# AnimatedRNG/alphazero-rs

Hardware: AMD Instinct MI355X
Metric: selfplay_games_per_sec (higher is better)
Workload: dtype bf16

## Files before the change

alphazero-rs_amd/csrc/az_net.hip:

```cpp
#include "az_net.h"
#include "az_fp8.h"

#include <algorithm>
#include <cmath>
#include <cstring>
#include <vector>

namespace az {

constexpr int ACTIONS = ConnectFour::ACTIONS;

typedef __bf16 bf16x8 __attribute__((ext_vector_type(8)));
typedef float f32x4 __attribute__((ext_vector_type(4)));
typedef int i32x4 __attribute__((ext_vector_type(4)));
typedef int i32x8 __attribute__((ext_vector_type(8)));

__global__ void k_net_fixture(EvalBatch eb, int kind, uint64_t salt) {
    uint32_t i = blockIdx.x * blockDim.x + threadIdx.x;
    if (i >= *eb.n) return;
    float pi[ACTIONS], v;
    if (kind == 0) {
#pragma unroll
        for (int a = 0; a < ACTIONS; ++a) pi[a] = __fdiv_rn(1.0f, 7.0f);
        v = 1.0f;
// ... 251 lines not shown
    const uint32_t b_off0 = (uint32_t)((n0 + srow) * d.K + chunk * 8), b_off1 = b_off0 + 32u * (uint32_t)d.K,
                   b_off2 = b_off0 + 64u * (uint32_t)d.K, b_off3 = b_off0 + 96u * (uint32_t)d.K;
    uint4 ra0, ra1, ra2, ra3, rb0, rb1, rb2, rb3;
#define AZ_GLOAD(kt_)                                                                           \
    {                                                                                           \
         \
        const int cb_ = (kt_) / ntaps, tap = (kt_) - cb_ * ntaps;                               \
        const int c0 = cb_ * GBK, kk = tap * d.cin + c0;                                        \
        const int ky = tap / d.tap_w, kx = tap - ky * d.tap_w;                                  \
        const uint32_t toff = (uint32_t)((ky * d.in_w + kx) * d.in_c + c0);                     \
        ra0 = *(const uint4*)(d.A + a_off0 + toff); ra1 = *(const uint4*)(d.A + a_off1 + toff); \
        ra2 = *(const uint4*)(d.A + a_off2 + toff); ra3 = *(const uint4*)(d.A + a_off3 + toff); \
        rb0 = *(const uint4*)(d.W + b_off0 + kk); rb1 = *(const uint4*)(d.W + b_off1 + kk);     \
        rb2 = *(const uint4*)(d.W + b_off2 + kk); rb3 = *(const uint4*)(d.W + b_off3 + kk);     \
    }
#define AZ_SWRITE(buf_)                                                                         \
    {                                                                                           \
        unsigned char* sa_ = smem[buf_] + tid * 16;                                             \
        unsigned char* sb_ = sa_ + GBM * 128;                                                   \
        *(uint4*)(sa_) = ra0; *(uint4*)(sa_ + 4096) = ra1; *(uint4*)(sa_ + 8192) = ra2; *(uint4*)(sa_ + 12288) = ra3; \
        *(uint4*)(sb_) = rb0; *(uint4*)(sb_ + 4096) = rb1; *(uint4*)(sb_ + 8192) = rb2; *(uint4*)(sb_ + 12288) = rb3; \
    }
    f32x4 acc[4][4];
#pragma unroll
    for (int i = 0; i < 4; ++i)
#pragma unroll
        for (int jn = 0; jn < 4; ++jn) acc[i][jn] = f32x4{0.f, 0.f, 0.f, 0.f};
    const int nk = d.K / GBK;
    const int frow = lane & 15, fq = lane >> 4, fsw = lane & 7;
    AZ_GLOAD(0);
    AZ_SWRITE(0);
    __syncthreads();
    for (int kt = 0; kt < nk; ++kt) {
        if (kt + 1 < nk) AZ_GLOAD(kt + 1);
        const unsigned char* sA = smem[kt & 1];
        const unsigned char* sB = sA + GBM * 128;
#pragma unroll
        for (int ks = 0; ks < 2; ++ks) {
            const int coff = ((ks * 4 + fq) ^ fsw) << 4;
            bf16x8 fa[4], fb[4];
#pragma unroll
            for (int mt = 0; mt < 4; ++mt) fa[mt] = *(const bf16x8*)(sA + (wr * 64 + mt * 16 + frow) * 128 + coff);
#pragma unroll
            for (int nt = 0; nt < 4; ++nt) fb[nt] = *(const bf16x8*)(sB + (wc * 64 + nt * 16 + frow) * 128 + coff);
#pragma unroll
            for (int mt = 0; mt < 4; ++mt)
#pragma unroll
                for (int nt = 0; nt < 4; ++nt)
                    acc[mt][nt] = __builtin_amdgcn_mfma_f32_16x16x32_bf16(fb[nt], fa[mt], acc[mt][nt], 0, 0, 0);
        }
        if (kt + 1 < nk) AZ_SWRITE((kt + 1) & 1);
        __syncthreads();
    }
#undef AZ_GLOAD
#undef AZ_SWRITE
#pragma unroll
    for (int nt = 0; nt < 4; ++nt) {
        const int n = n0 + wc * 64 + nt * 16 + fq * 4;
        const float4 bv = d.out_f16 ? make_float4(0.f, 0.f, 0.f, 0.f) : *(const float4*)(d.bias + n);
#pragma unroll
        for (int mt = 0; mt < 4; ++mt) {
            const int m = m0 + wr * 64 + mt * 16 + frow;
            if (m >= M) continue;
            float r0 = acc[mt][nt][0] + bv.x, r1 = acc[mt][nt][1] + bv.y, r2 = acc[mt][nt][2] + bv.z,
                  r3 = acc[mt][nt][3] + bv.w;
            if (d.relu) { r0 = fmaxf(r0, 0.f); r1 = fmaxf(r1, 0.f); r2 = fmaxf(r2, 0.f); r3 = fmaxf(r3, 0.f); }
            uint2 o;
            if (d.out_f16) {
                o.x = pack_f16x2(r0, r1);
                o.y = pack_f16x2(r2, r3);
            } else {
                o.x = pack_bf16x2(r0, r1);
                o.y = pack_bf16x2(r2, r3);
            }
            *(uint2*)(d.out + (size_t)m * d.N + n) = o;
        }
    }
}

__device__ __forceinline__ void lds_dma16(const void* sbase , uint32_t voff, uint32_t lds_addr ) {
    asm volatile("s_mov_b32 m0, %2\n\ts_nop 0\n\tglobal_load_lds_dwordx4 %0, %1" ::"v"(voff), "s"(sbase), "s"(lds_addr) : "memory");
}

template <int NS, int BM, int F8 = 0>
__device__ __forceinline__ void gemm_ring_body(const GemmDesc& d, unsigned char* smem , const int M) {
    static_assert(BM % 32 == 0 && BM >= 64 && BM <= 192 && NS * (BM * 128 + 16384) <= 163840 && 2 * (BM / 32 + 4) <= 63, "tile");
    constexpr int ES = F8 ? 1 : 2;
    constexpr int KB = 128 / ES;
    constexpr int MT = BM / 32;
    constexpr int STAGE = BM * 128 + 16384;
    constexpr int NDMA = MT + 4;
    const int ntaps = d.K / d.cin;
    const int NT = d.N / GBN;
    const int id = blockIdx.x;
    const int xcd = id & 7, j = id >> 3;
    const int ntile = j % NT, mtile = (j / NT) * 8 + xcd;
    const int m0 = mtile * BM, n0 = ntile * GBN;
    if (m0 >= M) return;
    const int tid = threadIdx.x, lane = tid & 63;
    const int wave = __builtin_amdgcn_readfirstlane(tid >> 6);
    const int wr = wave >> 1, wc = wave & 1;
    const int lrow = lane >> 3;
    const int chunk = (lane & 7) ^ lrow;
    uint32_t a_ob[MT];
#pragma unroll
    for (int q = 0; q < MT; ++q) {
        int m = m0 + (q * 4 + wave) * 8 + lrow;
        m = m < M ? m : M - 1;
        const int b = m / d.rows_per_sample, r = m - b * d.rows_per_sample;
        const int y = r / d.out_w, x = r - y * d.out_w;
        a_ob[q] = (uint32_t)(((b * d.in_h + y) * d.in_w + x) * d.in_c + chunk * (16 / ES)) * (uint32_t)ES;
    }
    const bool packed = F8 || d.Wr != nullptr;
    const uint32_t b_ob = packed ? (uint32_t)(wave * 1024 + lane * 16)
                                 : (uint32_t)((n0 + wave * 8 + lrow) * d.K + chunk * 8) * 2u;
    const size_t w_stride = packed ? (size_t)4096 : (size_t)64 * d.K;
    const char* wr_tile = (const char*)d.Wr + (size_t)ntile * (size_t)(d.K / KB) * 16384;
    int ks_idx = 0;
    typedef __attribute__((address_space(3))) void* lds_ptr;
    const uint32_t lds0 = (uint32_t)(uintptr_t)(lds_ptr)(smem + wave * 1024);
    int ks_tap = 0, ks_kx = 0;
    uint32_t ks_c0 = 0, ks_toff = 0, ks_kk = 0;
#define AZ_RDMA(buf_)                                                                                   \
    {                                                                                                   \
        const char* abase = (const char*)d.A + (size_t)ks_toff * ES;                                    \
        const char* wbase = packed ? wr_tile + (size_t)ks_idx * 16384 : (const char*)(d.W + ks_kk);     \
        ++ks_idx;                                                                                       \
        const uint32_t la = lds0 + (buf_) * STAGE;                                                      \
        _Pragma("unroll") for (int q_ = 0; q_ < MT; ++q_) lds_dma16(abase, a_ob[q_], la + q_ * 4096);   \
        _Pragma("unroll") for (int q_ = 0; q_ < 4; ++q_) lds_dma16(wbase + q_ * w_stride, b_ob, la + BM * 128 + q_ * 4096); \
        ++ks_tap; ++ks_kx; ks_toff += (uint32_t)d.in_c; ks_kk += (uint32_t)d.cin;                       \
        if (ks_kx == d.tap_w) { ks_kx = 0; ks_toff += (uint32_t)((d.in_w - d.tap_w) * d.in_c); }        \
        if (ks_tap == ntaps) { ks_tap = 0; ks_kx = 0; ks_c0 += KB; ks_toff = ks_c0; ks_kk = ks_c0; }    \
    }
    f32x4 acc[MT][4];
#pragma unroll
    for (int i = 0; i < MT; ++i)
#pragma unroll
        for (int jn = 0; jn < 4; ++jn) acc[i][jn] = f32x4{0.f, 0.f, 0.f, 0.f};
    const int nk = d.K / KB;
    const int frow = lane & 15, fq = lane >> 4, fsw = lane & 7;
#pragma unroll
    for (int st = 0; st < NS - 1; ++st)
        if (st < nk) AZ_RDMA(st);
    for (int kt = 0; kt < nk; ++kt) {
        const int younger = nk - 1 - kt < NS - 2 ? nk - 1 - kt : NS - 2;
        if (younger >= 2) asm volatile("s_waitcnt vmcnt(%0)" ::"n"(2 * NDMA) : "memory");
        else if (younger == 1) asm volatile("s_waitcnt vmcnt(%0)" ::"n"(NDMA) : "memory");
        else asm volatile("s_waitcnt vmcnt(0)" ::: "memory");
        __builtin_amdgcn_s_barrier();
        __builtin_amdgcn_sched_barrier(0);
        if (kt + NS - 1 < nk) AZ_RDMA((kt + NS - 1) % NS);
        const unsigned char* sA = smem + (kt % NS) * STAGE;
        const unsigned char* sB = sA + BM * 128;
        const int coff0 = ((0 + fq) ^ fsw) << 4, coff1 = ((4 + fq) ^ fsw) << 4;
        if constexpr (F8) {
            i32x8 fa[MT], fb[4];
#pragma unroll
            for (int nt = 0; nt < 4; ++nt) {
                const unsigned char* row = sB + (wc * 64 + nt * 16 + frow) * 128;
                fb[nt] = __builtin_shufflevector(*(const i32x4*)(row + coff0), *(const i32x4*)(row + coff1), 0, 1, 2, 3, 4, 5, 6, 7);
            }
#pragma unroll
            for (int mt = 0; mt < MT; ++mt) {
                const unsigned char* row = sA + (wr * (BM / 2) + mt * 16 + frow) * 128;
                fa[mt] = __builtin_shufflevector(*(const i32x4*)(row + coff0), *(const i32x4*)(row + coff1), 0, 1, 2, 3, 4, 5, 6, 7);
            }
#pragma unroll
            for (int mt = 0; mt < MT; ++mt)
#pragma unroll
                for (int nt = 0; nt < 4; ++nt)
                    acc[mt][nt] = __builtin_amdgcn_mfma_scale_f32_16x16x128_f8f6f4(fb[nt], fa[mt], acc[mt][nt], 0, 0, 0, 0, 0, 0);
            __builtin_amdgcn_sched_barrier(0);
            continue;
        }
        bf16x8 fa0[MT], fb0[4], fa1[MT], fb1[4];
#pragma unroll
        for (int mt = 0; mt < MT; ++mt) fa0[mt] = *(const bf16x8*)(sA + (wr * (BM / 2) + mt * 16 + frow) * 128 + coff0);
#pragma unroll
        for (int nt = 0; nt < 4; ++nt) fb0[nt] = *(const bf16x8*)(sB + (wc * 64 + nt * 16 + frow) * 128 + coff0);
#pragma unroll
        for (int mt = 0; mt < MT; ++mt) fa1[mt] = *(const bf16x8*)(sA + (wr * (BM / 2) + mt * 16 + frow) * 128 + coff1);
#pragma unroll
        for (int nt = 0; nt < 4; ++nt) fb1[nt] = *(const bf16x8*)(sB + (wc * 64 + nt * 16 + frow) * 128 + coff1);
#pragma unroll
        for (int mt = 0; mt < MT; ++mt)
#pragma unroll
            for (int nt = 0; nt < 4; ++nt)
                acc[mt][nt] = __builtin_amdgcn_mfma_f32_16x16x32_bf16(fb0[nt], fa0[mt], acc[mt][nt], 0, 0, 0);
#pragma unroll
        for (int mt = 0; mt < MT; ++mt)
#pragma unroll
            for (int nt = 0; nt < 4; ++nt)
                acc[mt][nt] = __builtin_amdgcn_mfma_f32_16x16x32_bf16(fb1[nt], fa1[mt], acc[mt][nt], 0, 0, 0);
        __builtin_amdgcn_sched_group_barrier(0x100, MT + 4, 0);
#pragma unroll
        for (int g = 0; g < MT + 4; ++g) {
            __builtin_amdgcn_sched_group_barrier(0x008, 1, 0);
            __builtin_amdgcn_sched_group_barrier(0x100, 1, 0);
        }
        __builtin_amdgcn_sched_group_barrier(0x008, 8 * MT - (MT + 4), 0);
        __builtin_amdgcn_sched_barrier(0);
    }
#undef AZ_RDMA
    constexpr bool OUT8 = F8 == 1;
    constexpr int EP_STRIDE = OUT8 ? 144 : 272;
    static_assert(BM * EP_STRIDE <= NS * STAGE, "the output tile must fit the ring");
    __builtin_amdgcn_s_waitcnt(0xC07F);
    __builtin_amdgcn_s_barrier();
#pragma unroll
    for (int nt = 0; nt < 4; ++nt) {
        const int nl = wc * 64 + nt * 16 + fq * 4;
        const float4 bv = *(const float4*)(d.bias + n0 + nl);
        float4 qv = make_float4(1.f, 1.f, 1.f, 1.f);
        if constexpr (F8 != 0) qv = *(const float4*)(d.dq + n0 + nl);
#pragma unroll
        for (int mt = 0; mt < MT; ++mt) {
            const int ml = wr * (BM / 2) + mt * 16 + frow;
            float r0 = acc[mt][nt][0], r1 = acc[mt][nt][1], r2 = acc[mt][nt][2], r3 = acc[mt][nt][3];
            if constexpr (F8 != 0) { r0 *= qv.x; r1 *= qv.y; r2 *= qv.z; r3 *= qv.w; }
            r0 += bv.x; r1 += bv.y; r2 += bv.z; r3 += bv.w;
            if (d.relu) { r0 = fmaxf(r0, 0.f); r1 = fmaxf(r1, 0.f); r2 = fmaxf(r2, 0.f); r3 = fmaxf(r3, 0.f); }
            if constexpr (OUT8) {
                *(uint32_t*)(smem + ml * EP_STRIDE + nl) = pack_fp8x4(r0, r1, r2, r3, d.out_scale);
            } else {
                uint2 o;
                o.x = pack_bf16x2(r0, r1);
                o.y = pack_bf16x2(r2, r3);
                *(uint2*)(smem + ml * EP_STRIDE + nl * 2) = o;
            }
        }
    }
    __syncthreads();
    constexpr int ROW16 = OUT8 ? 8 : 16;
#pragma unroll
    for (int it = 0; it < BM * ROW16 / 256; ++it) {
        const int idx = it * 256 + tid;
        const int ml = idx / ROW16, c = idx % ROW16;
        const int m = m0 + ml;
        if (m >= M) continue;
        *(uint4*)((unsigned char*)d.out + ((size_t)m * d.N + n0) * (OUT8 ? 1 : 2) + c * 16) = *(const uint4*)(smem + ml * EP_STRIDE + c * 16);
    }
}


AZ_HD int ring_pick_bm(int M, int ncol, int ns, bool conv) {
    auto wgs = [&](int bm) { return (M + bm - 1) / bm * ncol; };
    if (ns == 4) return wgs(64) <= 256 ? 64 : wgs(96) <= 256 ? 96 : 128;
    if (!conv) return wgs(96) <= 512 ? 96 : 128;
    int best = 128;
    float best_cost = 1e30f;
    for (int bm = 96; bm <= 192; bm += 32) {
        const int w = wgs(bm), full = w / 512, rem = w % 512;
        const float cost = (10.f + 0.42f * (float)bm) * ((float)full + (rem == 0 ? 0.f : rem <= 256 ? 0.6f : 1.f));
        if (cost < best_cost) { best_cost = cost; best = bm; }
    }
    return best;
}
template <int LAYER, int NS>
__global__ __launch_bounds__(256, (NS <= 2 ? 2 : 1)) void k_gemm_ring_auto(const GemmDesc d) {
    constexpr int BMAX = NS == 2 ? 192 : 128;
    __shared__ __attribute__((aligned(16))) unsigned char smem[NS * (BMAX * 128 + 16384)];
    const int M = (int)(*d.n_dev) * d.rows_per_sample;
    if (M <= d.m_min || (d.m_hi > 0 && M > d.m_hi)) return;
    const int bm = __builtin_amdgcn_readfirstlane(ring_pick_bm(M, d.N / GBN, NS, d.tap_w > 1));
    if constexpr (NS == 2) {
        if (bm == 96) gemm_ring_body<2, 96>(d, smem, M);
        else if (bm == 160) gemm_ring_body<2, 160>(d, smem, M);
        else if (bm == 192) gemm_ring_body<2, 192>(d, smem, M);
        else gemm_ring_body<2, 128>(d, smem, M);
    } else {
        if (bm == 64) gemm_ring_body<4, 64>(d, smem, M);
        else if (bm == 96) gemm_ring_body<4, 96>(d, smem, M);
        else gemm_ring_body<4, 128>(d, smem, M);
    }
}

template <int LAYER, int NS, int F8>
__global__ __launch_bounds__(256, (NS <= 2 ? 2 : 1)) void k_gemm_ring_f8(const GemmDesc d) {
    constexpr int BMAX = NS == 2 ? 192 : 128;
    __shared__ __attribute__((aligned(16))) unsigned char smem[NS * (BMAX * 128 + 16384)];
    const int M = (int)(*d.n_dev) * d.rows_per_sample;
    if (M <= d.m_min) return;
    const int bm = __builtin_amdgcn_readfirstlane(ring_pick_bm(M, d.N / GBN, NS, true));
    if constexpr (NS == 2) {
        if (bm == 96) gemm_ring_body<2, 96, F8>(d, smem, M);
        else if (bm == 160) gemm_ring_body<2, 160, F8>(d, smem, M);
        else if (bm == 192) gemm_ring_body<2, 192, F8>(d, smem, M);
        else gemm_ring_body<2, 128, F8>(d, smem, M);
    } else {
        if (bm == 64) gemm_ring_body<4, 64, F8>(d, smem, M);
        else if (bm == 96) gemm_ring_body<4, 96, F8>(d, smem, M);
        else gemm_ring_body<4, 128, F8>(d, smem, M);
    }
}

constexpr int HBN_ = 256;
constexpr int HBN2_ = 128;
constexpr int IMG_NB = 6;
constexpr int IMG_ROWS = IMG_NB * 42;
constexpr int IMG_ZERO_ROW = 252;

__device__ __forceinline__ void lds_dma16(const void* sbase, uint32_t voff, uint32_t lds_addr);
template <int LAYER, bool TABLE = false>
__global__ __launch_bounds__(256, 2) void k_conv_same_pipe(const GemmDesc d) {
    __shared__ __attribute__((aligned(16))) unsigned char smem[2 * 32768];
    const int n_boards = (int)(*d.n_dev);
    const int M = n_boards * 42;
    const int C = d.cin;
    const int NT = d.N / HBN2_;
    const int id = blockIdx.x;
    const int xcd = id & 7, j = id >> 3;
    const int ntile = j % NT, mtile = (j / NT) * 8 + xcd;
    const int b0 = mtile * IMG_NB, n0 = ntile * HBN2_;
    if (b0 >= n_boards) return;
    const int tid = threadIdx.x, lane = tid & 63;
    const int wave = __builtin_amdgcn_readfirstlane(tid >> 6);
    const int wr = wave >> 1, wc = wave & 1;
    if (tid < 8) *(uint4*)(smem + IMG_ZERO_ROW * 128 + tid * 16) = make_uint4(0, 0, 0, 0);
    const int lrow = lane >> 3;
    const int chunk = (lane & 7) ^ lrow;
    uint32_t i_ob[8];
#pragma unroll
    for (int q = 0; q < 8; ++q) {
        int r = (q * 4 + wave) * 8 + lrow;
        r = r < IMG_ROWS ? r : IMG_ROWS - 1;
        int b = b0 + r / 42;
        b = b < n_boards ? b : n_boards - 1;
        const int p = r % 42, y = p / 7, x = p - y * 7;
        if constexpr (TABLE) {
            const ulonglong2 st = d.states[b];
            i_ob[q] = (conv1_pattern(st.x, st.y, y, x) * (uint32_t)C + (uint32_t)chunk * 8u) * 2u;
        } else {
            i_ob[q] = (uint32_t)(((b * 8 + y + 1) * 9 + x + 1) * C + chunk * 8) * 2u;
        }
    }
    const bool i_last_ok = (7 * 4 + wave) * 8 + lrow < IMG_ROWS;
    const uint32_t w_ob = (uint32_t)((n0 + wave * 8 + lrow) * d.K + chunk * 8) * 2u;
    const size_t w_stride = (size_t)64 * d.K;
    typedef __attribute__((address_space(3))) void* lds_ptr;
    const uint32_t lds_img = (uint32_t)(uintptr_t)(lds_ptr)(smem + wave * 1024);
    const uint32_t lds_w = (uint32_t)(uintptr_t)(lds_ptr)(smem + 32768 + wave * 1024);
#define AZ_CDMA_W(kk_, buf_)                                                                                 \
    {                                                                                                        \
        const char* wbase = (const char*)(d.W + (kk_));                                                      \
        _Pragma("unroll") for (int q_ = 0; q_ < 4; ++q_) lds_dma16(wbase + q_ * w_stride, w_ob, lds_w + (buf_) * 16384 + q_ * 4096); \
    }
#define AZ_CDMA_IMG(cb_)                                                                                     \
    {                                                                                                        \
        const char* ibase = (const char*)(d.A + (cb_) * 64);                                                 \
        _Pragma("unroll") for (int q_ = 0; q_ < 7; ++q_) lds_dma16(ibase, i_ob[q_], lds_img + q_ * 4096);    \
        if (i_last_ok) lds_dma16(ibase, i_ob[7], lds_img + 7 * 4096);                                        \
    }
    f32x4 acc[8][4];
#pragma unroll
    for (int i = 0; i < 8; ++i)
#pragma unroll
        for (int jn = 0; jn < 4; ++jn) acc[i][jn] = f32x4{0.f, 0.f, 0.f, 0.f};
    const int frow = lane & 15, fq = lane >> 4, fsw = lane & 7;
    uint32_t rowmask[8];
#pragma unroll
    for (int mt = 0; mt < 8; ++mt) {
        const int ml = wr * 128 + mt * 16 + frow;
        const int p = ml % 42, y = p / 7, x = p - y * 7;
        uint32_t mask = 0;
#pragma unroll
        for (int t = 0; t < 9; ++t) {
            const int iy = y + t / 3 - 1, ix = x + t % 3 - 1;
            if (ml < IMG_ROWS && iy >= 0 && iy < 6 && ix >= 0 && ix < 7) mask |= 1u << t;
        }
        rowmask[mt] = (uint32_t)ml | (mask << 16);
    }
    const int b_row0 = 32768 + (wc * 64 + frow) * 128;
    const int coffB0 = ((0 + fq) ^ fsw) << 4, coffB1 = ((4 + fq) ^ fsw) << 4;
#define AZ_CLDA(dst_, mt0_, ks_, tap_, dtv_)                                                                 \
    _Pragma("unroll") for (int i_ = 0; i_ < 4; ++i_) {                                                       \
        const uint32_t rm_ = rowmask[(mt0_) + i_];                                                           \
// ... 893 lines not shown
            std::vector<uint16_t> wr((size_t)9 * C * C);
            for (int co = 0; co < C; ++co)
                for (int t = 0; t < 9; ++t)
                    std::memcpy(&wr[((size_t)t * C + co) * C], &w[(size_t)co * K[0] + (size_t)t * C], (size_t)C * 2);
            ok &= hipMemcpy(net->w2r, wr.data(), wr.size() * 2, hipMemcpyHostToDevice) == hipSuccess;
            GemmDesc d{};
            d.A = net->t1; d.W = net->w2r; d.bias = net->bg[0]; d.out = net->u2; d.n_dev = net->npat;
            d.rows_per_sample = 1; d.out_w = 1; d.in_h = 1; d.in_w = 1; d.in_c = C; d.tap_w = 1; d.cin = C; d.K = C; d.N = 9 * C;
            d.relu = 0; d.out_f16 = 1;
            const int mt8 = ((CONV1_PATTERNS + GBM - 1) / GBM + 7) / 8 * 8;
            hipLaunchKernelGGL(k_gemm_mfma<6>, dim3(mt8 * (d.N / GBN)), dim3(256), 0, nullptr, d);
            ok &= hipDeviceSynchronize() == hipSuccess;
        }
    }
    {
        std::vector<float> w(8 * 512), b(8);
        for (int k = 0; k < 512; ++k) {
            for (int a = 0; a < 7; ++a) w[(size_t)a * 512 + k] = p[L.pi_w + (int64_t)k * 7 + a];
            w[(size_t)7 * 512 + k] = p[L.v_w + k];
        }
        for (int a = 0; a < 7; ++a) b[a] = p[L.pi_b + a];
        b[7] = p[L.v_b];
        ok &= hipMemcpy(net->wh, w.data(), w.size() * 4, hipMemcpyHostToDevice) == hipSuccess;
        ok &= hipMemcpy(net->bh, b.data(), b.size() * 4, hipMemcpyHostToDevice) == hipSuccess;
    }
    return ok;
}

bool convnet_get_params(const ConvNet* n, float* host_params, int64_t count) {
    if (!n || (int64_t)n->params.size() != count) return false;
    std::memcpy(host_params, n->params.data(), (size_t)count * sizeof(float));
    return true;
}

void convnet_init_random(ConvNet* net, uint64_t seed) {
    const Layout L(net->C);
    const int C = net->C;
    std::vector<float> p((size_t)L.total, 0.0f);
    uint64_t ctr = 0;
    auto fill = [&](int64_t off, int64_t n, int fan_in, int fan_out) {
        const float lim = std::sqrt(6.0f / (float)(fan_in + fan_out));
        for (int64_t i = 0; i < n; ++i) {
            uint64_t r = rng_draw(seed, ctr++, 0, RNG_WEIGHTS);
            float u = (float)(uint32_t)(r >> 40) * (1.0f / 16777216.0f);
            p[(size_t)(off + i)] = (2.0f * u - 1.0f) * lim;
        }
    };
    auto bn_default = [&](int64_t off, int n) {
        for (int i = 0; i < n; ++i) { p[(size_t)(off + i)] = 1.0f; p[(size_t)(off + 3 * n + i)] = 1.0f; }
    };
    for (int l = 0; l < 4; ++l) {
        int cin = l == 0 ? 2 : C;
        fill(L.conv_w[l], 9ll * cin * C, 9 * cin, 9 * C);
        bn_default(L.conv_bn[l], C);
    }
    fill(L.fc_w[0], 6ll * C * 1024, 6 * C, 1024); bn_default(L.fc_bn[0], 1024);
    fill(L.fc_w[1], 1024ll * 512, 1024, 512); bn_default(L.fc_bn[1], 512);
    fill(L.pi_w, 512 * 7, 512, 7);
    fill(L.v_w, 512, 512, 1);
    convnet_set_params(net, p.data(), L.total);
}


static bool conv3_is_small(const GemmDesc& d, int rows_hint, int rows_typ) {
    return (rows_typ > 0 ? (long long)rows_typ * 115 / 100 : (long long)rows_hint) * d.rows_per_sample <= 8192;
}
template <bool TABLE>
static void launch_conv2_gemm(const GemmDesc& d, int rows_hint, hipStream_t s) {
    const int tiles = (rows_hint + IMG_NB - 1) / IMG_NB;
    const int t8 = (tiles + 7) / 8 * 8;
    hipLaunchKernelGGL((k_conv_same_pipe<1, TABLE>), dim3(t8 * (d.N / HBN2_)), dim3(256), 0, s, d);
}
static void launch_conv3_image(const GemmDesc& d, int rows_hint, hipStream_t s, bool tail, bool planes, bool wreg) {
    const int tiles = (rows_hint + C3_NB - 1) / C3_NB;
    const int t8 = (tiles + 7) / 8 * 8;
    const int full_grid = t8 * (d.N / 128), tail_wgs = tail ? C3_TAIL : 0;
    const dim3 grid(full_grid + tail_wgs), block(256);
    if (wreg && planes && d.Wf) hipLaunchKernelGGL((k_conv3_auto_wreg<2>), grid, block, 0, s, d, full_grid, tail_wgs);
    else if (planes) hipLaunchKernelGGL((k_conv3_auto<2, true>), grid, block, 0, s, d, full_grid, tail_wgs);
    else hipLaunchKernelGGL((k_conv3_auto<2, false>), grid, block, 0, s, d, full_grid, tail_wgs);
}

template <int LAYER, int F8 = 0>
static void launch_ring_auto(const GemmDesc& d, int rows_hint, int rows_typ, hipStream_t s, bool force_one_per_cu = false) {
    const int m_est = (int)((rows_typ > 0 ? (long long)rows_typ * 115 / 100 : (long long)rows_hint) * d.rows_per_sample), ncol = d.N / GBN;
    const bool conv = d.tap_w > 1;
    const int tile_max = conv ? 96 : 128;
    const int m_one = 256 / ncol * tile_max;
    const int m_bound = rows_hint * d.rows_per_sample;
    auto launch = [&](bool one_per_cu, const GemmDesc& dd, int m_cover) {
        const int bmin = one_per_cu ? 64 : 96;
        const int mtb = ((m_cover + bmin - 1) / bmin + 7) / 8 * 8;
        if constexpr (F8 != 0) {
            if (one_per_cu) hipLaunchKernelGGL((k_gemm_ring_f8<LAYER, 4, F8>), dim3(mtb * ncol), dim3(256), 0, s, dd);
            else hipLaunchKernelGGL((k_gemm_ring_f8<LAYER, 2, F8>), dim3(mtb * ncol), dim3(256), 0, s, dd);
        } else if (one_per_cu) hipLaunchKernelGGL((k_gemm_ring_auto<LAYER, 4>), dim3(mtb * ncol), dim3(256), 0, s, dd);
        else hipLaunchKernelGGL((k_gemm_ring_auto<LAYER, 2>), dim3(mtb * ncol), dim3(256), 0, s, dd);
    };
    if (!force_one_per_cu && !conv && m_bound > m_one && (long long)m_est * 100 >= (long long)m_one * 70 && (long long)m_est * 100 <= (long long)m_one * 140) {
        GemmDesc lo = d, hi = d;
        lo.m_hi = m_one;
        hi.m_min = std::max(d.m_min, m_one);
        launch(true, lo, std::min(m_bound, m_one));
        launch(false, hi, m_bound);
        return;
    }
    const bool one_per_cu = force_one_per_cu || m_bound <= m_one || (m_est + tile_max - 1) / tile_max * ncol <= 256;
    launch(one_per_cu, d, m_bound);
}

#ifdef AZ_DIAG
template <int LAYER>
static bool launch_gemm_diag(const GemmDesc& d, int rows_hint, int rows_typ, hipStream_t s, const NetOptions& o) {
    const int v = o.gemm_variant;
    if ((v == 3 || v == 5) && LAYER == 1 && d.N % HBN_ == 0 && d.cin % 64 == 0) {
        const int tiles = (rows_hint + IMG_NB - 1) / IMG_NB;
        const int t8 = (tiles + 7) / 8 * 8;
        if (v == 5 && o.conv2_pipe) return false;
        if (v == 5 && d.states) hipLaunchKernelGGL((k_conv_img2<LAYER, true>), dim3(t8 * (d.N / HBN2_)), dim3(256), 0, s, d);
        else if (v == 5) hipLaunchKernelGGL((k_conv_img2<LAYER>), dim3(t8 * (d.N / HBN2_)), dim3(256), 0, s, d);
        else hipLaunchKernelGGL((k_conv_img<LAYER>), dim3(t8 * (d.N / HBN_)), dim3(512), 0, s, d);
        return true;
    }
    const bool big = v >= 1 && (LAYER == 1 || LAYER == 2 || (LAYER == 3 && !o.ring_tile[3] && (o.conv4_big == 1 || (o.conv4_big == 2 && rows_typ >= 4096)))) &&
                     d.N % HBN_ == 0;
    if constexpr (LAYER == 2) if (v == 5 && o.conv3_ring) {
        const int mt = (rows_hint * d.rows_per_sample + GBM - 1) / GBM;
        const int mt8 = (mt + 7) / 8 * 8;
        if (o.conv3_ring == 3) launch_ring_auto<LAYER>(d, rows_hint, rows_typ, s, true);
        else if (o.conv3_ring == 2) hipLaunchKernelGGL((k_gemm_ring<LAYER, 4>), dim3(mt8 * (d.N / GBN)), dim3(256), 0, s, d);
        else hipLaunchKernelGGL((k_gemm_ring<LAYER, 2>), dim3(mt8 * (d.N / GBN)), dim3(256), 0, s, d);
        return true;
    }
    if constexpr (LAYER == 2) if (v == 5 && d.rows_per_sample == 20) {
        if ((o.conv3_small && conv3_is_small(d, rows_hint, rows_typ)) || o.conv3_pipe == 1) return false;
        const int tiles = (rows_hint + C3_NB - 1) / C3_NB;
        const int t8 = (tiles + 7) / 8 * 8;
        const dim3 g3(t8 * (d.N / 128)), b3(256);
        switch (o.conv3_pipe) {
            case 2: hipLaunchKernelGGL((k_conv_valid_pipe<LAYER, C3_NB, 6, 7, false, false>), g3, b3, 0, s, d); break;
            case 3: hipLaunchKernelGGL((k_conv_valid_pipe<LAYER, C3_NB, 6, 7, true, true>), g3, b3, 0, s, d); break;
            default: hipLaunchKernelGGL((k_conv_valid_img2<LAYER, C3_NB, 6, 7, 2>), g3, b3, 0, s, d); break;
        }
        return true;
    }
    if (v == 5 && !big && o.fc_ring == 1 && !(LAYER >= 3 && o.ring_tile[LAYER])) return false;
    if (big) {
        const int mt = (rows_hint * d.rows_per_sample + HBM_ - 1) / HBM_;
        const int mt8 = (mt + 7) / 8 * 8;
        const dim3 grid(mt8 * (d.N / HBN_)), block(512);
        if (v == 1) hipLaunchKernelGGL((k_gemm256<LAYER, 0>), grid, block, 0, s, d);
        else if (v == 13) hipLaunchKernelGGL((k_gemm256<LAYER, 1, true>), grid, block, 0, s, d);
        else hipLaunchKernelGGL((k_gemm256<LAYER, 1>), grid, block, 0, s, d);
        return true;
    }
    const int mt = (rows_hint * d.rows_per_sample + GBM - 1) / GBM;
    const int mt8 = (mt + 7) / 8 * 8;
    const int grid = mt8 * (d.N / GBN);
    if (v == 5 && o.fc_ring) {
        auto ring = [&](auto bm_c, auto ns_c) {
            constexpr int BM = decltype(bm_c)::value, NS = decltype(ns_c)::value;
            const int mtb = ((rows_hint * d.rows_per_sample + BM - 1) / BM + 7) / 8 * 8;
            hipLaunchKernelGGL((k_gemm_ring<LAYER, NS, BM>), dim3(mtb * (d.N / GBN)), dim3(256), 0, s, d);
        };
        using std::integral_constant;
        if constexpr (LAYER >= 3) {
            switch (o.ring_tile[LAYER]) {
                case 642: ring(integral_constant<int, 64>{}, integral_constant<int, 2>{}); return true;
                case 644: ring(integral_constant<int, 64>{}, integral_constant<int, 4>{}); return true;
                case 962: ring(integral_constant<int, 96>{}, integral_constant<int, 2>{}); return true;
                case 964: ring(integral_constant<int, 96>{}, integral_constant<int, 4>{}); return true;
                case 1282: ring(integral_constant<int, 128>{}, integral_constant<int, 2>{}); return true;
                case 1284: ring(integral_constant<int, 128>{}, integral_constant<int, 4>{}); return true;
                case 1602: ring(integral_constant<int, 160>{}, integral_constant<int, 2>{}); return true;
                case 1922: ring(integral_constant<int, 192>{}, integral_constant<int, 2>{}); return true;
                default: break;
            }
        }
        if (o.fc_ring == 2) {
            const int m_typ = (rows_typ > 0 ? rows_typ : rows_hint) * d.rows_per_sample, ncol = d.N / GBN;
            const bool conv = d.tap_w > 1;
            const int ns = (m_typ + (conv ? 95 : 127)) / (conv ? 96 : 128) * ncol <= 256 ? 4 : 2;
            switch (ring_pick_bm(m_typ, ncol, ns, conv) * 10 + ns) {
                case 644: ring(integral_constant<int, 64>{}, integral_constant<int, 4>{}); break;
                case 964: ring(integral_constant<int, 96>{}, integral_constant<int, 4>{}); break;
                case 1284: ring(integral_constant<int, 128>{}, integral_constant<int, 4>{}); break;
                case 962: ring(integral_constant<int, 96>{}, integral_constant<int, 2>{}); break;
                case 1602: ring(integral_constant<int, 160>{}, integral_constant<int, 2>{}); break;
                case 1922: ring(integral_constant<int, 192>{}, integral_constant<int, 2>{}); break;
                default: ring(integral_constant<int, 128>{}, integral_constant<int, 2>{}); break;
            }
            return true;
        }
        if (o.fc_ring == 1) return false;
        hipLaunchKernelGGL((k_gemm_ring<LAYER, 2>), dim3(grid), dim3(256), 0, s, d);
        return true;
    }
    hipLaunchKernelGGL(k_gemm_mfma<LAYER>, dim3(grid), dim3(256), 0, s, d);
    return true;
}
#endif

template <int LAYER>
static void launch_gemm(const GemmDesc& d, int rows_hint, int rows_typ, hipStream_t s, const NetOptions& o) {
#ifdef AZ_DIAG
    if (launch_gemm_diag<LAYER>(d, rows_hint, rows_typ, s, o)) return;
#endif
    GemmDesc dd = d;
    if constexpr (LAYER >= 2) if (o.narrow_rows > 0 && d.N % 32 == 0) {
        const int lim = o.narrow_rows * (LAYER == 2 ? 1 : LAYER == 3 ? 2 : 4);
        const int est = rows_typ > 0 ? rows_typ : rows_hint;
        if (est <= 16 * lim) {
            dd.m_max = lim * d.rows_per_sample;
            const int rows_cov = rows_hint < lim ? rows_hint : lim;
            const dim3 grid((unsigned)skinny_waves_max(rows_cov * d.rows_per_sample, d.N)), block(64);
            const int nk = d.K / GBK;
            if (nk % 8 == 0) hipLaunchKernelGGL((k_gemm_skinny<LAYER, 8>), grid, block, 0, s, dd);
            else if (nk % 6 == 0) hipLaunchKernelGGL((k_gemm_skinny<LAYER, 6>), grid, block, 0, s, dd);
            else hipLaunchKernelGGL((k_gemm_skinny<LAYER, 2>), grid, block, 0, s, dd);
            if (rows_hint <= lim) return;
            dd.m_min = dd.m_max;
        }
    }
    const GemmDesc& d2 = dd;
    if constexpr (LAYER == 1) if (d.N % HBN_ == 0 && d.cin % 64 == 0) {
        if (d.states) launch_conv2_gemm<true>(d2, rows_hint, s);
        else launch_conv2_gemm<false>(d2, rows_hint, s);
        return;
    }
    if constexpr (LAYER == 2) {
        if (o.conv3_small && conv3_is_small(d2, rows_hint, rows_typ)) launch_ring_auto<LAYER>(d2, rows_hint, rows_typ, s, true);
        else launch_conv3_image(d2, rows_hint, s, o.conv3_tail != 0, o.conv3_planes != 0, o.conv3_wreg != 0);
        return;
    }

    launch_ring_auto<LAYER>(d2, rows_hint, rows_typ, s);
}

template <int LAYER, int F8>
static void launch_gemm_f8(const GemmDesc& d, int rows_hint, int rows_typ, hipStream_t s, const NetOptions& o, NetWorkspace* ws) {
    GemmDesc dd = d;
    if (o.narrow_rows > 0 && d.N % 32 == 0 && d.cin % 128 == 0) {
        const int lim = o.narrow_rows * (LAYER == 2 ? 1 : 2);
        const int est = rows_typ > 0 ? rows_typ : rows_hint;
        if (est <= 16 * lim) {
            dd.m_max = lim * d.rows_per_sample;
            const int rows_cov = rows_hint < lim ? rows_hint : lim;
            const dim3 grid((unsigned)skinny_waves_max(rows_cov * d.rows_per_sample, d.N)), block(64);
// ... 324 lines not shown
```

alphazero-rs_amd/csrc/az_net_diag.inc:

```

typedef _Float16 f16x8 __attribute__((ext_vector_type(8)));
__global__ __launch_bounds__(256) void k_conv2_table(const EvalBatch eb, const uint16_t* __restrict__ U ,
                                                     const float* __restrict__ bias , uint16_t* __restrict__ out ,
                                                     int C) {
    extern __shared__ __attribute__((aligned(16))) unsigned char u0_lds[];
    for (int i = threadIdx.x; i < 9 * C / 8; i += blockDim.x) ((uint4*)u0_lds)[i] = ((const uint4*)U)[i];
    __syncthreads();
    const int lane = threadIdx.x & 63;
    const uint32_t items = *eb.n * 6u;
    const uint32_t wave0 = blockIdx.x * 4u + (threadIdx.x >> 6), nwaves = gridDim.x * 4u;
    const int cg = C / 8;
    for (uint32_t it = wave0; it < items; it += nwaves) {
        const uint32_t b = it / 6u;
        const int y = (int)(it - b * 6u);
        const ulonglong2 sv = eb.state[b];
        const int ly = y - 1 + (lane < 21 ? lane / 7 : 0), lx = lane < 21 ? lane % 7 : 0;
        const uint32_t mypat = (ly >= 0 && ly < 6) ? conv1_pattern(sv.x, sv.y, ly, lx) : 0u;
        for (int x = 0; x < 7; ++x) {
            uint32_t row[9];
#pragma unroll
            for (int t = 0; t < 9; ++t) {
                const int ky = t / 3, qy = y + ky - 1, qx = x + t % 3 - 1;
                const bool in = qy >= 0 && qy < 6 && qx >= 0 && qx < 7;
                const uint32_t pq = (uint32_t)__builtin_amdgcn_readlane((int)mypat, in ? ky * 7 + qx : 0);
                row[t] = in ? pq * 9u + (uint32_t)t : 0xFFFFFFFFu;
            }
            for (int c8 = lane; c8 < cg; c8 += 64) {
                f16x8 u[9];
#pragma unroll
                for (int t = 0; t < 9; ++t) {
                    if (row[t] == 0xFFFFFFFFu) continue;
                    if (row[t] < 9u) u[t] = *(const f16x8*)(u0_lds + ((size_t)row[t] * C + (size_t)c8 * 8) * 2);
                    else u[t] = *(const f16x8*)(U + ((size_t)row[t] * C + (size_t)c8 * 8));
                }
                float acc[8] = {0.f, 0.f, 0.f, 0.f, 0.f, 0.f, 0.f, 0.f};
#pragma unroll
                for (int t = 0; t < 9; ++t)
                    if (row[t] != 0xFFFFFFFFu) {
#pragma unroll
                        for (int i = 0; i < 8; ++i) acc[i] += (float)u[t][i];
                    }
                const float4 b0 = *(const float4*)(bias + c8 * 8), b1 = *(const float4*)(bias + c8 * 8 + 4);
                uint4 o;
                o.x = pack_bf16x2(fmaxf(acc[0] + b0.x, 0.f), fmaxf(acc[1] + b0.y, 0.f));
                o.y = pack_bf16x2(fmaxf(acc[2] + b0.z, 0.f), fmaxf(acc[3] + b0.w, 0.f));
                o.z = pack_bf16x2(fmaxf(acc[4] + b1.x, 0.f), fmaxf(acc[5] + b1.y, 0.f));
                o.w = pack_bf16x2(fmaxf(acc[6] + b1.z, 0.f), fmaxf(acc[7] + b1.w, 0.f));
                *(uint4*)(out + ((size_t)b * 42 + (size_t)(y * 7 + x)) * C + (size_t)c8 * 8) = o;
            }
        }
    }
}

template <int LAYER, int NS, int BM = 128>
__global__ __launch_bounds__(256, (NS <= 2 ? 2 : 1)) void k_gemm_ring(const GemmDesc d) {
    __shared__ __attribute__((aligned(16))) unsigned char smem[NS * (BM * 128 + 16384)];
    gemm_ring_body<NS, BM>(d, smem, (int)(*d.n_dev) * d.rows_per_sample);
}

constexpr int HBM_ = 256;
template <int LAYER, int PIPE, bool STAMP = false>
__global__ __launch_bounds__(512, 2) void k_gemm256(const GemmDesc d) {
    __shared__ __attribute__((aligned(16))) unsigned char smem[2 * (HBM_ + HBN_) * 128];
    const int M = (int)(*d.n_dev) * d.rows_per_sample;
    const int ntaps = d.K / d.cin;
    const int NT = d.N / HBN_;
    const int id = blockIdx.x;
    const int xcd = id & 7, j = id >> 3;
    const int ntile = j % NT, mtile = (j / NT) * 8 + xcd;
    const int m0 = mtile * HBM_, n0 = ntile * HBN_;
    if (m0 >= M) return;
    const int tid = threadIdx.x, lane = tid & 63;
    const int wave = __builtin_amdgcn_readfirstlane(tid >> 6);
    const int wr = wave >> 2, wc = wave & 3;
    const int lrow = lane >> 3;
    const int chunk = (lane & 7) ^ lrow;
    auto row_off = [&](int q) -> uint32_t {
        int m = m0 + (q * 8 + wave) * 8 + lrow;
        m = m < M ? m : M - 1;
        const int b = m / d.rows_per_sample, r = m - b * d.rows_per_sample;
        const int y = r / d.out_w, x = r - y * d.out_w;
        return (uint32_t)(((b * d.in_h + y) * d.in_w + x) * d.in_c + chunk * 8);
    };
    const uint32_t a_off0 = row_off(0), a_off1 = row_off(1), a_off2 = row_off(2), a_off3 = row_off(3);
    const uint32_t b_off0 = (uint32_t)((n0 + wave * 8 + lrow) * d.K + chunk * 8);
    const uint32_t b_step = 64u * (uint32_t)d.K;
    const uint32_t a_ob0 = a_off0 * 2u, a_ob1 = a_off1 * 2u, a_ob2 = a_off2 * 2u, a_ob3 = a_off3 * 2u;
    const uint32_t b_ob0 = b_off0 * 2u, b_ob1 = (b_off0 + b_step) * 2u, b_ob2 = (b_off0 + 2u * b_step) * 2u,
                   b_ob3 = (b_off0 + 3u * b_step) * 2u;
    typedef __attribute__((address_space(3))) void* lds_ptr;
    typedef const __attribute__((address_space(1))) void* gbl_ptr;
    int ks_tap = 0, ks_kx = 0;
    uint32_t ks_c0 = 0, ks_toff = 0, ks_kk = 0;
#define AZ_KSTEP_ADVANCE()                                                                              \
    {                                                                                                   \
        ++ks_tap; ++ks_kx; ks_toff += (uint32_t)d.in_c; ks_kk += (uint32_t)d.cin;                       \
        if (ks_kx == d.tap_w) { ks_kx = 0; ks_toff += (uint32_t)((d.in_w - d.tap_w) * d.in_c); }        \
        if (ks_tap == ntaps) { ks_tap = 0; ks_kx = 0; ks_c0 += GBK; ks_toff = ks_c0; ks_kk = ks_c0; }   \
    }
#define AZ_DMA(kt_, buf_)                                                                               \
    {                                                                                                   \
         \
        const char* abase = (const char*)(d.A + ks_toff);                                               \
        const char* wbase = (const char*)(d.W + ks_kk);                                                 \
        unsigned char* la = smem + (buf_) * 65536 + wave * 1024;                                        \
        unsigned char* lb = la + 32768;                                                                 \
        __builtin_amdgcn_global_load_lds((gbl_ptr)(abase + a_ob0), (lds_ptr)(la), 16, 0, 0);            \
        __builtin_amdgcn_global_load_lds((gbl_ptr)(abase + a_ob1), (lds_ptr)(la + 8192), 16, 0, 0);     \
        __builtin_amdgcn_global_load_lds((gbl_ptr)(abase + a_ob2), (lds_ptr)(la + 16384), 16, 0, 0);    \
        __builtin_amdgcn_global_load_lds((gbl_ptr)(abase + a_ob3), (lds_ptr)(la + 24576), 16, 0, 0);    \
        __builtin_amdgcn_global_load_lds((gbl_ptr)(wbase + b_ob0), (lds_ptr)(lb), 16, 0, 0);            \
        __builtin_amdgcn_global_load_lds((gbl_ptr)(wbase + b_ob1), (lds_ptr)(lb + 8192), 16, 0, 0);     \
        __builtin_amdgcn_global_load_lds((gbl_ptr)(wbase + b_ob2), (lds_ptr)(lb + 16384), 16, 0, 0);    \
        __builtin_amdgcn_global_load_lds((gbl_ptr)(wbase + b_ob3), (lds_ptr)(lb + 24576), 16, 0, 0);    \
        AZ_KSTEP_ADVANCE();                                                                             \
    }
    f32x4 acc[8][4];
#pragma unroll
    for (int i = 0; i < 8; ++i)
#pragma unroll
        for (int jn = 0; jn < 4; ++jn) acc[i][jn] = f32x4{0.f, 0.f, 0.f, 0.f};
    const int nk = d.K / GBK;
    const int frow = lane & 15, fq = lane >> 4, fsw = lane & 7;
    AZ_DMA(0, 0);
    asm volatile("s_waitcnt vmcnt(0)" ::: "memory");
    __syncthreads();
    unsigned long long st0 = 0, sr0 = 0;
    if constexpr (STAMP) { st0 = __builtin_amdgcn_s_memtime(); sr0 = __builtin_amdgcn_s_memrealtime(); }
    const int a_row0 = (wr * 128 + frow) * 128, b_row0 = 32768 + (wc * 64 + frow) * 128;
    const int coff0 = ((0 + fq) ^ fsw) << 4, coff1 = ((4 + fq) ^ fsw) << 4;
#define AZ_LDA(dst_, base_, mt0_, coff_)                                                     \
    _Pragma("unroll") for (int i_ = 0; i_ < 4; ++i_)                                         \
        dst_[i_] = *(const bf16x8*)((base_) + a_row0 + ((mt0_) + i_) * 2048 + (coff_));
#define AZ_LDB(dst_, base_, coff_)                                                           \
    _Pragma("unroll") for (int i_ = 0; i_ < 4; ++i_)                                         \
        dst_[i_] = *(const bf16x8*)((base_) + b_row0 + i_ * 2048 + (coff_));
#define AZ_MMA(mt0_, fb_, fa_)                                                               \
    _Pragma("unroll") for (int i_ = 0; i_ < 4; ++i_)                                         \
        _Pragma("unroll") for (int j_ = 0; j_ < 4; ++j_)                                     \
            acc[(mt0_) + i_][j_] = __builtin_amdgcn_mfma_f32_16x16x32_bf16(fb_[j_], fa_[i_], acc[(mt0_) + i_][j_], 0, 0, 0);
// ... 731 lines not shown
```

Before: 10150.

## Use 8-wave ring GEMM kernel for FC layers in one-per-CU path

Adds a 512-thread (8-wave) variant of the ring-buffered bf16 GEMM in which each wave computes a 32-column slice instead of 64. It is now the default for layers 4 and up when one block per CU is chosen, with an optional late-refill schedule. The goal is more latency hiding and DMA issue parallelism per CU on the fully connected layers. The cost is more sync across waves and fewer MFMAs per wave between barriers. Diagnostic timestamp variants are also added behind template flags.

```diff
diff --git a/alphazero-rs_amd/csrc/az_net.hip b/alphazero-rs_amd/csrc/az_net.hip
--- a/alphazero-rs_amd/csrc/az_net.hip
+++ b/alphazero-rs_amd/csrc/az_net.hip
@@ -357,7 +357,7 @@
     asm volatile("s_mov_b32 m0, %2\n\ts_nop 0\n\tglobal_load_lds_dwordx4 %0, %1" ::"v"(voff), "s"(sbase), "s"(lds_addr) : "memory");
 }
 
-template <int NS, int BM, int F8 = 0>
+template <int NS, int BM, int F8 = 0, bool STAMP = false>
 __device__ __forceinline__ void gemm_ring_body(const GemmDesc& d, unsigned char* smem , const int M) {
     static_assert(BM % 32 == 0 && BM >= 64 && BM <= 192 && NS * (BM * 128 + 16384) <= 163840 && 2 * (BM / 32 + 4) <= 63, "tile");
     constexpr int ES = F8 ? 1 : 2;
@@ -418,6 +418,15 @@
 #pragma unroll
     for (int st = 0; st < NS - 1; ++st)
         if (st < nk) AZ_RDMA(st);
+    [[maybe_unused]] unsigned long long seg[4] = {0, 0, 0, 0}, tprev = 0, t_begin = 0, r_begin = 0;
+    if constexpr (STAMP) { t_begin = tprev = __builtin_amdgcn_s_memtime(); r_begin = __builtin_amdgcn_s_memrealtime(); }
+#define AZ_RSTAMP(i_)                                                                                   \
+    if constexpr (STAMP) {                                                                              \
+        __builtin_amdgcn_sched_barrier(0);                                                              \
+        const unsigned long long t_ = __builtin_amdgcn_s_memtime();                                     \
+        seg[i_] += t_ - tprev; tprev = t_;                                                              \
+        __builtin_amdgcn_sched_barrier(0);                                                              \
+    }
     for (int kt = 0; kt < nk; ++kt) {
         const int younger = nk - 1 - kt < NS - 2 ? nk - 1 - kt : NS - 2;
         if (younger >= 2) asm volatile("s_waitcnt vmcnt(%0)" ::"n"(2 * NDMA) : "memory");
@@ -425,7 +434,9 @@
         else asm volatile("s_waitcnt vmcnt(0)" ::: "memory");
         __builtin_amdgcn_s_barrier();
         __builtin_amdgcn_sched_barrier(0);
+        AZ_RSTAMP(0);
         if (kt + NS - 1 < nk) AZ_RDMA((kt + NS - 1) % NS);
+        AZ_RSTAMP(1);
         const unsigned char* sA = smem + (kt % NS) * STAGE;
         const unsigned char* sB = sA + BM * 128;
         const int coff0 = ((0 + fq) ^ fsw) << 4, coff1 = ((4 + fq) ^ fsw) << 4;
@@ -454,6 +465,7 @@
         for (int mt = 0; mt < MT; ++mt) fa0[mt] = *(const bf16x8*)(sA + (wr * (BM / 2) + mt * 16 + frow) * 128 + coff0);
 #pragma unroll
         for (int nt = 0; nt < 4; ++nt) fb0[nt] = *(const bf16x8*)(sB + (wc * 64 + nt * 16 + frow) * 128 + coff0);
+        AZ_RSTAMP(2);
 #pragma unroll
         for (int mt = 0; mt < MT; ++mt) fa1[mt] = *(const bf16x8*)(sA + (wr * (BM / 2) + mt * 16 + frow) * 128 + coff1);
 #pragma unroll
@@ -468,7 +480,7 @@
 #pragma unroll
             for (int nt = 0; nt < 4; ++nt)
                 acc[mt][nt] = __builtin_amdgcn_mfma_f32_16x16x32_bf16(fb1[nt], fa1[mt], acc[mt][nt], 0, 0, 0);
-        __builtin_amdgcn_sched_group_barrier(0x100, MT + 4, 0);
+        if constexpr (!STAMP) __builtin_amdgcn_sched_group_barrier(0x100, MT + 4, 0);
 #pragma unroll
         for (int g = 0; g < MT + 4; ++g) {
             __builtin_amdgcn_sched_group_barrier(0x008, 1, 0);
@@ -476,8 +488,17 @@
         }
         __builtin_amdgcn_sched_group_barrier(0x008, 8 * MT - (MT + 4), 0);
         __builtin_amdgcn_sched_barrier(0);
-    }
+        AZ_RSTAMP(3);
+    }
+#undef AZ_RSTAMP
 #undef AZ_RDMA
+    if constexpr (STAMP) {
+        if (tid == 0 && d.dbg && blockIdx.x < 128) {
+            for (int i = 0; i < 8; ++i) d.dbg[16 * blockIdx.x + i] = i < 4 ? seg[i] : 0ull;
+            d.dbg[16 * blockIdx.x + 8] = __builtin_amdgcn_s_memtime() - t_begin;
+            d.dbg[16 * blockIdx.x + 9] = __builtin_amdgcn_s_memrealtime() - r_begin;
+        }
+    }
     constexpr bool OUT8 = F8 == 1;
     constexpr int EP_STRIDE = OUT8 ? 144 : 272;
     static_assert(BM * EP_STRIDE <= NS * STAGE, "the output tile must fit the ring");
@@ -568,6 +589,176 @@
         else if (bm == 96) gemm_ring_body<4, 96, F8>(d, smem, M);
         else gemm_ring_body<4, 128, F8>(d, smem, M);
     }
+}
+
+template <int BM, bool LATE, bool STAMP = false>
+__device__ __forceinline__ void gemm_ring8_body(const GemmDesc& d, unsigned char* smem , const int M) {
+    static_assert(BM == 64 || BM == 96 || BM == 128, "tile");
+    constexpr int NS = 4;
+    constexpr int MT = BM / 32;
+    constexpr int STAGE = BM * 128 + 16384;
+    constexpr int APW = BM / 64;
+    constexpr bool ODD = BM % 64 != 0;
+    constexpr int NA = APW + (ODD ? 1 : 0);
+    const int NT = d.N / GBN;
+    const int id = blockIdx.x;
+    const int xcd = id & 7, j = id >> 3;
+    const int ntile = j % NT, mtile = (j / NT) * 8 + xcd;
+    const int m0 = mtile * BM, n0 = ntile * GBN;
+    if (m0 >= M) return;
+    const int tid = threadIdx.x, lane = tid & 63;
+    const int wave = __builtin_amdgcn_readfirstlane(tid >> 6);
+    const int wr = wave >> 2, wc = wave & 3;
+    const bool extra = ODD && wave < 4;
+    const bool late = LATE && wave >= 4;
+    const int lrow = lane >> 3;
+    const int chunk = (lane & 7) ^ lrow;
+    uint32_t a_ob[NA];
+#pragma unroll
+    for (int q = 0; q < NA; ++q) {
+        int m = m0 + (q * 8 + wave) * 8 + lrow;
+        m = m < M ? m : M - 1;
+        a_ob[q] = (uint32_t)(m * d.in_c + chunk * 8) * 2u;
+    }
+    const bool packed = d.Wr != nullptr;
+    const uint32_t b_ob = packed ? (uint32_t)(wave * 1024 + lane * 16)
+                                 : (uint32_t)((n0 + wave * 8 + lrow) * d.K + chunk * 8) * 2u;
+    const size_t w_stride = packed ? (size_t)8192 : (size_t)128 * d.K;
+    const char* wr_tile = (const char*)d.Wr + (size_t)ntile * (size_t)(d.K / 64) * 16384;
+    int ks_idx = 0;
+    typedef __attribute__((address_space(3))) void* lds_ptr;
+    const uint32_t lds0 = (uint32_t)(uintptr_t)(lds_ptr)(smem + wave * 1024);
+#define AZ_RDMA8(buf_)                                                                                  \
+    {                                                                                                   \
+        const char* abase = (const char*)d.A + (size_t)ks_idx * 128;                                    \
+        const char* wbase = packed ? wr_tile + (size_t)ks_idx * 16384 : (const char*)d.W + (size_t)ks_idx * 128; \
+        ++ks_idx;                                                                                       \
+        const uint32_t la = lds0 + (buf_) * STAGE;                                                      \
+        _Pragma("unroll") for (int q_ = 0; q_ < APW; ++q_) lds_dma16(abase, a_ob[q_], la + q_ * 8192);  \
+        if constexpr (ODD) if (extra) lds_dma16(abase, a_ob[APW], la + APW * 8192);                     \
+        _Pragma("unroll") for (int q_ = 0; q_ < 2; ++q_) lds_dma16(wbase + q_ * w_stride, b_ob, la + BM * 128 + q_ * 8192); \
+    }
+#define AZ_RWAIT8(N_)                                                                                   \
+    {                                                                                                   \
+        if (younger >= 2) asm volatile("s_waitcnt vmcnt(%0)" ::"n"(2 * (N_)) : "memory");               \
+        else if (younger == 1) asm volatile("s_waitcnt vmcnt(%0)" ::"n"(N_) : "memory");                \
+        else asm volatile("s_waitcnt vmcnt(0)" ::: "memory");                                           \
+    }
+    f32x4 acc[MT][2];
+#pragma unroll
+    for (int i = 0; i < MT; ++i)
+#pragma unroll
+        for (int jn = 0; jn < 2; ++jn) acc[i][jn] = f32x4{0.f, 0.f, 0.f, 0.f};
+    const int nk = d.K / 64;
+    const int frow = lane & 15, fq = lane >> 4, fsw = lane & 7;
+#pragma unroll
+    for (int st = 0; st < NS - 1; ++st)
+        if (st < nk) AZ_RDMA8(st);
+    [[maybe_unused]] unsigned long long seg[4] = {0, 0, 0, 0}, tprev = 0, t_begin = 0, r_begin = 0;
+    if constexpr (STAMP) { t_begin = tprev = __builtin_amdgcn_s_memtime(); r_begin = __builtin_amdgcn_s_memrealtime(); }
+#define AZ_RSTAMP(i_)                                                                                   \
+    if constexpr (STAMP) {                                                                              \
+        __builtin_amdgcn_sched_barrier(0);                                                              \
+        const unsigned long long t_ = __builtin_amdgcn_s_memtime();                                     \
+        seg[i_] += t_ - tprev; tprev = t_;                                                              \
+        __builtin_amdgcn_sched_barrier(0);                                                              \
+    }
+    for (int kt = 0; kt < nk; ++kt) {
+        const int younger = nk - 1 - kt < NS - 2 ? nk - 1 - kt : NS - 2;
+        if (extra) AZ_RWAIT8(APW + 3) else AZ_RWAIT8(APW + 2)
+        __builtin_amdgcn_s_barrier();
+        __builtin_amdgcn_sched_barrier(0);
+        AZ_RSTAMP(0);
+        const bool refill = kt + NS - 1 < nk;
+        if (refill && !late) AZ_RDMA8((kt + NS - 1) % NS);
+        AZ_RSTAMP(1);
+        const unsigned char* sA = smem + (kt % NS) * STAGE;
+        const unsigned char* sB = sA + BM * 128;
+        const int coff0 = ((0 + fq) ^ fsw) << 4, coff1 = ((4 + fq) ^ fsw) << 4;
+        bf16x8 fa0[MT], fb0[2], fa1[MT], fb1[2];
+#pragma unroll
+        for (int mt = 0; mt < MT; ++mt) fa0[mt] = *(const bf16x8*)(sA + (wr * (BM / 2) + mt * 16 + frow) * 128 + coff0);
+#pragma unroll
+        for (int nt = 0; nt < 2; ++nt) fb0[nt] = *(const bf16x8*)(sB + (wc * 32 + nt * 16 + frow) * 128 + coff0);
+        AZ_RSTAMP(2);
+#pragma unroll
+        for (int mt = 0; mt < MT; ++mt) fa1[mt] = *(const bf16x8*)(sA + (wr * (BM / 2) + mt * 16 + frow) * 128 + coff1);
+#pragma unroll
+        for (int nt = 0; nt < 2; ++nt) fb1[nt] = *(const bf16x8*)(sB + (wc * 32 + nt * 16 + frow) * 128 + coff1);
+#pragma unroll
+        for (int mt = 0; mt < MT; ++mt)
+#pragma unroll
+            for (int nt = 0; nt < 2; ++nt)
+                acc[mt][nt] = __builtin_amdgcn_mfma_f32_16x16x32_bf16(fb0[nt], fa0[mt], acc[mt][nt], 0, 0, 0);
+        if constexpr (!STAMP) __builtin_amdgcn_sched_group_barrier(0x100, MT + 2, 0);
+#pragma unroll
+        for (int g = 0; g < MT + 2; ++g) {
+            __builtin_amdgcn_sched_group_barrier(0x008, 1, 0);
+            __builtin_amdgcn_sched_group_barrier(0x100, 1, 0);
+        }
+        if constexpr (MT > 2) __builtin_amdgcn_sched_group_barrier(0x008, 2 * MT - (MT + 2), 0);
+        __builtin_amdgcn_sched_barrier(0);
+        if constexpr (LATE) if (refill && late) AZ_RDMA8((kt + NS - 1) % NS);
+        __builtin_amdgcn_sched_barrier(0);
+#pragma unroll
+        for (int mt = 0; mt < MT; ++mt)
+#pragma unroll
+            for (int nt = 0; nt < 2; ++nt)
+                acc[mt][nt] = __builtin_amdgcn_mfma_f32_16x16x32_bf16(fb1[nt], fa1[mt], acc[mt][nt], 0, 0, 0);
+        __builtin_amdgcn_sched_barrier(0);
+        AZ_RSTAMP(3);
+    }
+#undef AZ_RSTAMP
+#undef AZ_RDMA8
+#undef AZ_RWAIT8
+    if constexpr (STAMP) {
+        if ((tid == 0 || tid == 256) && d.dbg && blockIdx.x < 128) {
+            for (int i = 0; i < 4; ++i) d.dbg[16 * blockIdx.x + (tid >> 6) + i] = seg[i];
+            if (tid == 0) {
+                d.dbg[16 * blockIdx.x + 8] = __builtin_amdgcn_s_memtime() - t_begin;
+                d.dbg[16 * blockIdx.x + 9] = __builtin_amdgcn_s_memrealtime() - r_begin;
+            }
+        }
+    }
+    constexpr int EP_STRIDE = 272;
+    __builtin_amdgcn_s_waitcnt(0xC07F);
+    __builtin_amdgcn_s_barrier();
+#pragma unroll
+    for (int nt = 0; nt < 2; ++nt) {
+        const int nl = wc * 32 + nt * 16 + fq * 4;
+        const float4 bv = *(const float4*)(d.bias + n0 + nl);
+#pragma unroll
+        for (int mt = 0; mt < MT; ++mt) {
+            const int ml = wr * (BM / 2) + mt * 16 + frow;
+            float r0 = acc[mt][nt][0] + bv.x, r1 = acc[mt][nt][1] + bv.y, r2 = acc[mt][nt][2] + bv.z, r3 = acc[mt][nt][3] + bv.w;
+            if (d.relu) { r0 = fmaxf(r0, 0.f); r1 = fmaxf(r1, 0.f); r2 = fmaxf(r2, 0.f); r3 = fmaxf(r3, 0.f); }
+            uint2 o;
+            o.x = pack_bf16x2(r0, r1);
+            o.y = pack_bf16x2(r2, r3);
+            *(uint2*)(smem + ml * EP_STRIDE + nl * 2) = o;
+        }
+    }
+    __syncthreads();
+#pragma unroll
+    for (int it = 0; it < BM * 16 / 512; ++it) {
+        const int idx = it * 512 + tid;
+        const int ml = idx / 16, c = idx % 16;
+        const int m = m0 + ml;
+        if (m >= M) continue;
+        *(uint4*)((unsigned char*)d.out + ((size_t)m * d.N + n0) * 2 + c * 16) = *(const uint4*)(smem + ml * EP_STRIDE + c * 16);
+    }
+}
+
+constexpr int RING8_SHIPPED = 8;
+template <int LAYER, bool LATE>
+__global__ __launch_bounds__(512, 1) void k_gemm_ring8_auto(const GemmDesc d) {
+    __shared__ __attribute__((aligned(16))) unsigned char smem[4 * (128 * 128 + 16384)];
+    const int M = (int)(*d.n_dev) * d.rows_per_sample;
+    if (M <= d.m_min || (d.m_hi > 0 && M > d.m_hi)) return;
+    const int bm = __builtin_amdgcn_readfirstlane(ring_pick_bm(M, d.N / GBN, 4, false));
+    if (bm == 64) gemm_ring8_body<64, LATE>(d, smem, M);
+    else if (bm == 96) gemm_ring8_body<96, LATE>(d, smem, M);
+    else gemm_ring8_body<128, LATE>(d, smem, M);
 }
 
 constexpr int HBN_ = 256;
@@ -1627,7 +1818,7 @@
 }
 
 template <int LAYER, int F8 = 0>
-static void launch_ring_auto(const GemmDesc& d, int rows_hint, int rows_typ, hipStream_t s, bool force_one_per_cu = false) {
+static void launch_ring_auto(const GemmDesc& d, int rows_hint, int rows_typ, hipStream_t s, bool force_one_per_cu = false, int fc_waves = RING8_SHIPPED) {
     const int m_est = (int)((rows_typ > 0 ? (long long)rows_typ * 115 / 100 : (long long)rows_hint) * d.rows_per_sample), ncol = d.N / GBN;
     const bool conv = d.tap_w > 1;
     const int tile_max = conv ? 96 : 128;
@@ -1639,8 +1830,15 @@
         if constexpr (F8 != 0) {
             if (one_per_cu) hipLaunchKernelGGL((k_gemm_ring_f8<LAYER, 4, F8>), dim3(mtb * ncol), dim3(256), 0, s, dd);
             else hipLaunchKernelGGL((k_gemm_ring_f8<LAYER, 2, F8>), dim3(mtb * ncol), dim3(256), 0, s, dd);
-        } else if (one_per_cu) hipLaunchKernelGGL((k_gemm_ring_auto<LAYER, 4>), dim3(mtb * ncol), dim3(256), 0, s, dd);
-        else hipLaunchKernelGGL((k_gemm_ring_auto<LAYER, 2>), dim3(mtb * ncol), dim3(256), 0, s, dd);
+        } else if (one_per_cu) {
+            if constexpr (LAYER >= 4) {
+#ifdef AZ_DIAG
+                if (fc_waves == 4) { hipLaunchKernelGGL((k_gemm_ring_auto<LAYER, 4>), dim3(mtb * ncol), dim3(256), 0, s, dd); return; }
+                if (fc_waves != RING8_SHIPPED) { hipLaunchKernelGGL((k_gemm_ring8_auto<LAYER, RING8_SHIPPED != 9>), dim3(mtb * ncol), dim3(512), 0, s, dd); return; }
+#endif
+                hipLaunchKernelGGL((k_gemm_ring8_auto<LAYER, RING8_SHIPPED == 9>), dim3(mtb * ncol), dim3(512), 0, s, dd);
+            } else hipLaunchKernelGGL((k_gemm_ring_auto<LAYER, 4>), dim3(mtb * ncol), dim3(256), 0, s, dd);
+        } else hipLaunchKernelGGL((k_gemm_ring_auto<LAYER, 2>), dim3(mtb * ncol), dim3(256), 0, s, dd);
     };
     if (!force_one_per_cu && !conv && m_bound > m_one && (long long)m_est * 100 >= (long long)m_one * 70 && (long long)m_est * 100 <= (long long)m_one * 140) {
         GemmDesc lo = d, hi = d;
@@ -1709,6 +1907,16 @@
             hipLaunchKernelGGL((k_gemm_ring<LAYER, NS, BM>), dim3(mtb * (d.N / GBN)), dim3(256), 0, s, d);
         };
         using std::integral_constant;
+        if constexpr (LAYER >= 4) {
+            const int code = o.ring_tile[LAYER];
+            if (code == 4 || code == 8 || code == 9) { launch_ring_auto<LAYER>(d, rows_hint, rows_typ, s, false, code); return true; }
+            if (code == 5 || code == 6) {
+                const int mtb = ((rows_hint * d.rows_per_sample + 63) / 64 + 7) / 8 * 8;
+                if (code == 5) hipLaunchKernelGGL((k_gemm_ring_stamp<LAYER>), dim3(mtb * (d.N / GBN)), dim3(256), 0, s, d);
+                else hipLaunchKernelGGL((k_gemm_ring8_stamp<LAYER>), dim3(mtb * (d.N / GBN)), dim3(512), 0, s, d);
+                return true;
+            }
+        }
         if constexpr (LAYER >= 3) {
             switch (o.ring_tile[LAYER]) {
                 case 642: ring(integral_constant<int, 64>{}, integral_constant<int, 2>{}); return true;
diff --git a/alphazero-rs_amd/csrc/az_net_diag.inc b/alphazero-rs_amd/csrc/az_net_diag.inc
--- a/alphazero-rs_amd/csrc/az_net_diag.inc
+++ b/alphazero-rs_amd/csrc/az_net_diag.inc
@@ -56,6 +56,26 @@
 __global__ __launch_bounds__(256, (NS <= 2 ? 2 : 1)) void k_gemm_ring(const GemmDesc d) {
     __shared__ __attribute__((aligned(16))) unsigned char smem[NS * (BM * 128 + 16384)];
     gemm_ring_body<NS, BM>(d, smem, (int)(*d.n_dev) * d.rows_per_sample);
+}
+
+template <int LAYER>
+__global__ __launch_bounds__(256, 1) void k_gemm_ring_stamp(const GemmDesc d) {
+    __shared__ __attribute__((aligned(16))) unsigned char smem[4 * (128 * 128 + 16384)];
+    const int M = (int)(*d.n_dev) * d.rows_per_sample;
+    const int bm = __builtin_amdgcn_readfirstlane(ring_pick_bm(M, d.N / GBN, 4, d.tap_w > 1));
+    if (bm == 64) gemm_ring_body<4, 64, 0, true>(d, smem, M);
+    else if (bm == 96) gemm_ring_body<4, 96, 0, true>(d, smem, M);
+    else gemm_ring_body<4, 128, 0, true>(d, smem, M);
+}
+
+template <int LAYER>
+__global__ __launch_bounds__(512, 1) void k_gemm_ring8_stamp(const GemmDesc d) {
+    __shared__ __attribute__((aligned(16))) unsigned char smem[4 * (128 * 128 + 16384)];
+    const int M = (int)(*d.n_dev) * d.rows_per_sample;
+    const int bm = __builtin_amdgcn_readfirstlane(ring_pick_bm(M, d.N / GBN, 4, false));
+    if (bm == 64) gemm_ring8_body<64, RING8_SHIPPED == 9, true>(d, smem, M);
+    else if (bm == 96) gemm_ring8_body<96, RING8_SHIPPED == 9, true>(d, smem, M);
+    else gemm_ring8_body<128, RING8_SHIPPED == 9, true>(d, smem, M);
 }
 
 constexpr int HBM_ = 256;
```

New measurement: 10260, median of 6. No clear change (+1.0%).
